# marian42/shapegan

Measured on AMD Instinct MI355X. Metric: GAN train steps/sec @32^3 voxels (train_wgan.py 5 critic + 1 generator updates, batch 64/GPU), higher is better.
Workload: dtype f32; 1 GPU; train_wgan.py 32^3 voxel WGAN, fp32, batch=64 synthetic SDF grids (BASELINE configs[1]); global_batch=64, per_gpu_batch=64, parallelism=dp1

## Files before the change

### shapegan_amd/csrc/conv3d.hip

```cpp
#include "mfma_tile.h"
#include <stdlib.h>

#include "conv_common.h"
#include "../../include/shapegan_hip.h"

namespace sg {

struct PatchCtx {
    int base;
    int mask;
    __device__ __forceinline__ void set(const ConvGeom& g, uint32_t pos) {
        int n, od, oh, ow;
        decode_pos(g, pos, n, od, oh, ow);
        const int id0 = 2 * od - 1, ih0 = 2 * oh - 1, iw0 = 2 * ow - 1;
        base = n * g.Cx * g.ID * g.IH * g.IW + (id0 * g.IH + ih0) * g.IW + iw0;
        int m = 0;
#pragma unroll
        for (int t = 0; t < 4; ++t) {
            if ((unsigned)(id0 + t) < (unsigned)g.ID) m |= 1 << t;
            if ((unsigned)(ih0 + t) < (unsigned)g.IH) m |= 1 << (4 + t);
            if ((unsigned)(iw0 + t) < (unsigned)g.IW) m |= 1 << (8 + t);
        }
        mask = m;
    }
// ... 655 lines not shown
                      false);
}
int sg_conv3d_k4s2p1_dgrad_keep(const float* dy, const float* w, const float* bias, float* dx, int batch, int Cin,
                                int Cin_total, int Cx, int Cout, int ID, int IH, int IW, int act, float slope,
                                void* workspace, size_t workspace_bytes, int weights_unchanged, hipStream_t stream) {
    return dgrad_call(dy, w, bias, dx, batch, Cin, Cin_total, Cx, Cout, ID, IH, IW, act, slope, workspace, workspace_bytes, stream,
                      weights_unchanged != 0);
}

int sg_conv3d_k4s2p1_pack_images(int n, const int* kinds, const float* const* weights, void* const* workspaces,
                                 const size_t* workspace_bytes, const int* dims, int* served, hipStream_t stream) {
    SG_CHECK_ARG(n > 0 && n <= 8 && kinds && weights && workspaces && workspace_bytes && dims && served);
    PackJobs jobs;
    static const float dummy = 0.f;
    for (int i = 0; i < n; ++i) {
        const int* d = dims + 8 * i;
        const int batch = d[0], Cin = d[1], Cin_total = d[2], Cx = d[3], Cout = d[4];
        served[i] = 0;
        SG_CHECK_ARG(weights[i] && batch > 0 && Cin > 0 && Cin <= Cin_total && Cin <= Cx && Cout > 0 && (kinds[i] == 0 || kinds[i] == 1));
        ConvGeom g;
        if (make_geom(g, d[5], d[6], d[7], Cx, Cout)) SG_FAIL(SG_ERR_ARG, "sg_conv3d_k4s2p1_pack_images: bad spatial dims");
        if (check_sizes(g, batch, "sg_conv3d_k4s2p1_pack_images")) return SG_ERR_ARG;
        if (Cin == 1) continue;
        int rc;
        if (kinds[i] == 0)
            rc = halo_fwd_try(&dummy, weights[i], nullptr, const_cast<float*>(&dummy), batch, Cin, Cin_total, g, Cout, SG_ACT_NONE, 0.f,
                              workspaces[i], workspace_bytes[i], stream, 0, 0, false, &jobs);
        else
            rc = halo_dgrad_try(&dummy, weights[i], nullptr, const_cast<float*>(&dummy), batch, Cin, Cin_total, g, Cout, SG_ACT_NONE, 0.f,
                                workspaces[i], workspace_bytes[i], stream, 0, false, &jobs);
        if (rc < 0) return rc;
        served[i] = rc == 1;
    }
    halo_pack_jobs_launch(jobs, stream);
    SG_CHECK_LAUNCH();
    return SG_OK;
}

long long sg_conv3d_k4s2p1_image_layout(int kind, const int* dims, size_t workspace_bytes) {
    if (!dims || (kind != 0 && kind != 1)) return 0;
    const int batch = dims[0], Cin = dims[1], Cin_total = dims[2], Cx = dims[3], Cout = dims[4];
    if (batch <= 0 || Cin <= 1 || Cin > Cin_total || Cin > Cx || Cout <= 0) return 0;
    ConvGeom g;
    if (make_geom(g, dims[5], dims[6], dims[7], Cx, Cout)) return 0;
    if ((long)batch * g.O3() >= (1L << 31) || (long)batch * g.I3() >= (1L << 31)) return 0;
    PackJobs jobs;
    static const float dummy = 0.f;
    char* const base = reinterpret_cast<char*>(uintptr_t(1) << 20);
    const int rc = kind == 0 ? halo_fwd_try(&dummy, &dummy, nullptr, const_cast<float*>(&dummy), batch, Cin, Cin_total, g, Cout, SG_ACT_NONE,
                                            0.f, base, workspace_bytes, nullptr, 0, 0, false, &jobs)
                             : halo_dgrad_try(&dummy, &dummy, nullptr, const_cast<float*>(&dummy), batch, Cin, Cin_total, g, Cout,
                                              SG_ACT_NONE, 0.f, base, workspace_bytes, nullptr, 0, false, &jobs);
    if (rc != 1 || jobs.n != 1) return 0;
    const PackJob& j = jobs.job[0];
    unsigned long long h = 1469598103934665603ull;
    const long long f[7] = {j.kind + 1, j.Cout, j.Cin_total, j.Cin, j.nt, (long long)(reinterpret_cast<char*>(j.wp) - base), 0x5347};
    for (long long v : f)
        for (int b = 0; b < 8; ++b) {
            h ^= (unsigned long long)(v >> (8 * b)) & 0xffull;
            h *= 1099511628211ull;
        }
    h &= 0x7fffffffffffffffull;
    return h ? (long long)h : 1;
}

int sg_conv3d_k4s2p1_dgrad_impl(const float* dy, const float* w, const float* bias, float* dx, int batch, int Cin,
                                int Cin_total, int Cx, int Cout, int ID, int IH, int IW, int act, float slope,
                                void* workspace, size_t workspace_bytes, int impl, hipStream_t stream) {
    SG_CHECK_ARG(dy && w && dx && batch > 0 && Cin > 0 && Cin <= Cin_total && Cin <= Cx && Cout > 0 && (impl & 1) &&
                 (impl == 1 || impl == 3 || impl == 9 || impl == 17 || impl == 33));
    ConvGeom g;
    if (make_geom(g, ID, IH, IW, Cx, Cout)) SG_FAIL(SG_ERR_ARG, "sg_conv3d_k4s2p1_dgrad_impl: bad spatial dims");
    if (check_sizes(g, batch, "sg_conv3d_k4s2p1_dgrad_impl")) return SG_ERR_ARG;
    const int rc = halo_dgrad_try(dy, w, bias, dx, batch, Cin, Cin_total, g, Cout, act, slope, workspace, workspace_bytes,
                                  stream, impl);
    if (rc != 1) SG_FAIL(SG_ERR_ARG, "sg_conv3d_k4s2p1_dgrad_impl: shape not eligible for the LDS-halo kernel");
    SG_CHECK_LAUNCH();
    return SG_OK;
}

int sg_conv3d_k4s2p1_wgrad_impl(const float* dy, const float* x, float* dw, int batch, int Cin, int Cin_total, int Cx,
                                int Cout, int ID, int IH, int IW, void* workspace, size_t workspace_bytes, int impl,
                                hipStream_t stream) {
    SG_CHECK_ARG(dy && x && dw && batch > 0 && Cin > 0 && Cin <= Cin_total && Cin <= Cx && Cout > 0 && impl == 1);
    ConvGeom g;
    if (make_geom(g, ID, IH, IW, Cx, Cout)) SG_FAIL(SG_ERR_ARG, "sg_conv3d_k4s2p1_wgrad_impl: bad spatial dims");
    if (check_sizes(g, batch, "sg_conv3d_k4s2p1_wgrad_impl")) return SG_ERR_ARG;
    const int rc = halo_wgrad_try(dy, x, dw, batch, Cin, Cin_total, g, Cout, workspace, workspace_bytes, stream, 1);
    if (rc != 1) SG_FAIL(SG_ERR_ARG, "sg_conv3d_k4s2p1_wgrad_impl: shape not eligible for the LDS-halo kernel");
    SG_CHECK_LAUNCH();
    return SG_OK;
}

int sg_conv3d_k4s2p1_wgrad_dy_image(int batch, int Cin, int Cout, int OD, int OH, int OW, size_t workspace_bytes, int* mt_total,
                                    long* nslice) {
    if (batch <= 0 || Cin <= 0 || Cout <= 0 || !mt_total || !nslice) return 0;
    ConvGeom g;
    if (make_geom(g, 2 * OD, 2 * OH, 2 * OW, Cin, Cout)) return 0;
    if (Cin == 1 && Cout <= 64) return 0;
    return halo_wgrad_dy_image_plan(batch, Cin, Cout, g, workspace_bytes, mt_total, nslice);
}
int sg_act_bwd_rowsum_pack8(const float* y, const float* dy, float* dz, float* rowsum, void* dz_image, long N, int C, long nslice,
                            int act, float slope, hipStream_t stream) {
    SG_CHECK_ARG(y && dy && dz && rowsum && dz_image && N > 0 && C > 0 && C % 128 == 0 && nslice == N * 8);
    SG_CHECK_ARG(act == SG_ACT_LEAKY || act == SG_ACT_RELU);
    SG_CHECK_ARG((((uintptr_t)y | (uintptr_t)dy | (uintptr_t)dz | (uintptr_t)dz_image) & 15) == 0);
    halo_act_bwd_pack8_launch(y, dy, dz, rowsum, dz_image, N * C, C, nslice, act, slope, stream);
    SG_CHECK_LAUNCH();
    return SG_OK;
}
int sg_conv3d_k4s2p1_wgrad_prepacked(const float* dy, const float* x, float* dw, int batch, int Cin, int Cin_total, int Cx,
                                     int Cout, int ID, int IH, int IW, void* workspace, size_t workspace_bytes, hipStream_t stream) {
    SG_CHECK_ARG(dy && x && dw && batch > 0 && Cin > 0 && Cin <= Cin_total && Cin <= Cx && Cout > 0);
    ConvGeom g;
    if (make_geom(g, ID, IH, IW, Cx, Cout)) SG_FAIL(SG_ERR_ARG, "sg_conv3d_k4s2p1_wgrad_prepacked: bad spatial dims");
    if (check_sizes(g, batch, "sg_conv3d_k4s2p1_wgrad_prepacked")) return SG_ERR_ARG;
    int mt;
    long ns;
    if (!halo_wgrad_dy_image_plan(batch, Cin, Cout, g, workspace_bytes, &mt, &ns))
        SG_FAIL(SG_ERR_ARG, "sg_conv3d_k4s2p1_wgrad_prepacked: this call is not served with a producer-written image");
    if (halo_wgrad_try(dy, x, dw, batch, Cin, Cin_total, g, Cout, workspace, workspace_bytes, stream, 0, true) != 1)
        SG_FAIL(SG_ERR_ARG, "sg_conv3d_k4s2p1_wgrad_prepacked: not served");
    SG_CHECK_LAUNCH();
    return SG_OK;
}

int sg_conv3d_k4s2p1_wgrad_act_eligible(int batch, int Cin, int Cout, int OD, int OH, int OW, int act) {
    const size_t x_bytes = ((size_t)batch * 8 * OD * OH * OW + (size_t)(2 * OH + 1) * 2 * OW + 4) * 4;
    const size_t dy_bytes = (size_t)batch * Cout * OD * OH * OW * 4;
    return Cin == 1 && Cout <= 64 && OW % 16 == 0 && (long)batch * OD * OH * OW >= 65536 && (act == SG_ACT_LEAKY || act == SG_ACT_RELU) &&
           x_bytes < (size_t)kBufRange && dy_bytes < (size_t)kBufRange && edge_enabled(4);
}
int sg_conv3d_k4s2p1_wgrad_act(const float* dy, const float* y, const float* x, float* dw, float* db, int batch, int Cin,
                               int Cin_total, int Cx, int Cout, int ID, int IH, int IW, int act, float slope, void* workspace,
                               size_t workspace_bytes, hipStream_t stream) {
    SG_CHECK_ARG(dy && y && x && dw && db && batch > 0 && Cin > 0 && Cin <= Cin_total && Cin <= Cx && Cout > 0);
    ConvGeom g;
    if (make_geom(g, ID, IH, IW, Cx, Cout)) SG_FAIL(SG_ERR_ARG, "sg_conv3d_k4s2p1_wgrad_act: spatial dims must be even and >= 2");
    if (check_sizes(g, batch, "sg_conv3d_k4s2p1_wgrad_act")) return SG_ERR_ARG;
    if (!sg_conv3d_k4s2p1_wgrad_act_eligible(batch, Cin, Cout, g.OD, g.OH, g.OW, act) ||
        edge_wgrad_try(dy, x, dw, batch, Cin, Cin_total, g, Cout, workspace, workspace ? workspace_bytes : 0, stream, 0, y, act, slope,
                       db) != 1)
        SG_FAIL(SG_ERR_ARG, "sg_conv3d_k4s2p1_wgrad_act: shape not served (see sg_conv3d_k4s2p1_wgrad_act_eligible) or workspace too small");
    SG_CHECK_LAUNCH();
    return SG_OK;
}

int sg_conv3d_k4s2p1_wgrad(const float* dy, const float* x, float* dw, int batch, int Cin, int Cin_total, int Cx,
                           int Cout, int ID, int IH, int IW, void* workspace, size_t workspace_bytes,
                           hipStream_t stream) {
    SG_CHECK_ARG(dy && x && dw && batch > 0 && Cin > 0 && Cin <= Cin_total && Cin <= Cx && Cout > 0);
    ConvGeom g;
    if (make_geom(g, ID, IH, IW, Cx, Cout)) SG_FAIL(SG_ERR_ARG, "sg_conv3d_k4s2p1_wgrad: spatial dims must be even and >= 2");
    if (check_sizes(g, batch, "sg_conv3d_k4s2p1_wgrad")) return SG_ERR_ARG;
    const long npos = (long)batch * g.O3();
    if (Cin == 1 && edge_enabled(4) &&
        edge_wgrad_try(dy, x, dw, batch, Cin, Cin_total, g, Cout, workspace, workspace ? workspace_bytes : 0, stream) == 1) {
        SG_CHECK_LAUNCH();
        return SG_OK;
    }
    {
        const int rc = halo_wgrad_try(dy, x, dw, batch, Cin, Cin_total, g, Cout, workspace, workspace ? workspace_bytes : 0,
                                      stream, 0);
        if (rc < 0) return rc;
        if (rc == 1) {
            SG_CHECK_LAUNCH();
            return SG_OK;
        }
    }
    WgradDyLoader la;
    la.dy = dy;
// ... 69 lines not shown
```

### shapegan_amd/csrc/conv3d_halo.hip

```cpp
#include "conv_common.h"

#ifndef SG_RING
#define SG_RING 8
#endif
#ifndef SG_ABLATE
#define SG_ABLATE 0
#endif

namespace sg {

constexpr int kHD = 4, kHH = 18, kHWF = 18;
constexpr int kHWH = 10;
constexpr int kROWH = 2 * kHWH;
constexpr int kROWD = kHH * kROWH;
constexpr int kHS = kHD * kROWD;
constexpr int kCC = 4;

struct HaloFwdArgs {
    const float* x;
    const float4* wp;
    const float* bias;
    float* y;
    ConvGeom g;
    int Cin, Cout;
// ... 1038 lines not shown
                for (int t = 0; t < 2; ++t) a_cur[t] = aring[gq][t];
                int gi = (st + 1) * 8 + gq;
                gi = gi < G ? gi : G - 1;
#pragma unroll
                for (int t = 0; t < 2; ++t) aring[gq][t] = buf_load4(ares[t], avoff, (unsigned)gi * 1024u);
                float b[2][4];
#pragma unroll
                for (int tn = 0; tn < 2; ++tn)
#pragma unroll
                    for (int j = 0; j < 4; ++j) b[tn][j] = bq[tn][j];
                if (gq + 1 < 8) {
#pragma unroll
                    for (int tn = 0; tn < 2; ++tn) {
                        const lds_float* hb = bb[CUR][tn][(gq + 1) >> 2] + 2 * ((gq + 1) & 3) * kROWH;
                        bq[tn][0] = hb[0];
                        bq[tn][1] = hb[2];
                        bq[tn][2] = hb[4];
                        bq[tn][3] = hb[6];
                    }
                }
#pragma unroll
                for (int f = 0; f < NF; ++f) {
                    if (f * 4 / NF == gq) fv[f] = copy_load(f);
                    if (f * 4 / NF + 4 == gq) sdst[f % (kWNF / 2)][NXT * (NCH * kWHS) + (f / (kWNF / 2)) * kWHS] = fv[f];
                }
                __builtin_amdgcn_sched_barrier(0);
#pragma unroll
                for (int j = 0; j < 4; ++j) {
                    const float a0 = j == 0 ? a_cur[0].x : (j == 1 ? a_cur[0].y : (j == 2 ? a_cur[0].z : a_cur[0].w));
                    const float a1 = j == 0 ? a_cur[1].x : (j == 1 ? a_cur[1].y : (j == 2 ? a_cur[1].z : a_cur[1].w));
                    acc[0][0] = __builtin_amdgcn_mfma_f32_32x32x2f32(a0, b[0][j], acc[0][0], 0, 0, 0);
                    acc[1][0] = __builtin_amdgcn_mfma_f32_32x32x2f32(a1, b[0][j], acc[1][0], 0, 0, 0);
                    acc[0][1] = __builtin_amdgcn_mfma_f32_32x32x2f32(a0, b[1][j], acc[0][1], 0, 0, 0);
                    acc[1][1] = __builtin_amdgcn_mfma_f32_32x32x2f32(a1, b[1][j], acc[1][1], 0, 0, 0);
                }
                __builtin_amdgcn_sched_barrier(0);
            }
            __syncthreads();
        };
        for (int st = 0; st + 1 < nst; st += 2) {
            stage(IntTag<0>(), st);
            stage(IntTag<1>(), st + 1);
        }
        if (nst & 1) stage(IntTag<0>(), nst - 1);
    }

    float* out = a.ws + (long)split * a.Cout * a.ldw;
#pragma unroll
    for (int tn = 0; tn < 2; ++tn) {
        const int col = wn * 64 + tn * 32 + r;
        const int ci = ci0 + (col >> 6);
        if (ci >= a.Cin) continue;
        const long cbase = (long)ci * 64 + (col & 63);
#pragma unroll
        for (int t = 0; t < 2; ++t) {
#pragma unroll
            for (int q = 0; q < 16; ++q) {
                const int co = (mt0 + wm * 2 + t) * 32 + (q & 3) + 8 * (q >> 2) + 4 * kpar;
                if (co < a.Cout) out[(long)co * a.ldw + cbase] = acc[t][tn][q];
            }
        }
    }
}

__global__ void __launch_bounds__(256) pack_wgrad_dy4_kernel(const float* __restrict__ dy, float4* __restrict__ ap, int Cout,
                                                             int MT, int nslice) {
    const long total = (long)MT * nslice * 8 * 64;
    for (long e = (long)blockIdx.x * 256 + threadIdx.x; e < total; e += (long)gridDim.x * 256) {
        const int lane = (int)(e & 63);
        const int gq = (int)((e >> 6) & 7);
        const long q = e >> 9;
        const long sl = q % nslice;
        const int mt = (int)(q / nslice);
        const int co = mt * 32 + (lane & 31);
        float4 v = make_float4(0.f, 0.f, 0.f, 0.f);
        if (co < Cout) {
            const float* src = dy + (sl * Cout + co) * 64 + (gq >> 1) * 16 + (gq & 1) * 8 + (lane >> 5);
            v = make_float4(src[0], src[2], src[4], src[6]);
        }
        ap[e] = v;
    }
}

__global__ void __launch_bounds__(256) conv_wgrad_halo4_kernel(HaloWgradArgs a) {
    constexpr int kBUF = 2 * k4CH;
    extern __shared__ __attribute__((aligned(16))) float wbox[];
    lds_float* const wl = (lds_float*)wbox;
    const int tid = threadIdx.x, lane = tid & 63;
    const int wave = __builtin_amdgcn_readfirstlane(tid >> 6);
    const int wm = wave >> 1, wn = wave & 1, r = lane & 31, kpar = lane >> 5;
    const int ci0 = blockIdx.x * 2, mt0 = blockIdx.y * 4, split = blockIdx.z;
    const int s_beg = split * a.per_split, s_end = min(a.nslice, s_beg + a.per_split);
    const int nst = s_end - s_beg;

    f32x16 acc[2][2];
#pragma unroll
    for (int i = 0; i < 2; ++i)
#pragma unroll
        for (int j = 0; j < 2; ++j)
#pragma unroll
            for (int q = 0; q < 16; ++q) acc[i][j][q] = 0.f;

    for (int e = tid; e < 2 * kBUF; e += 256) wl[e] = 0.f;

    if (nst > 0) {
        const lds_float* bb[2][2][4];
#pragma unroll
        for (int tn = 0; tn < 2; ++tn) {
            const int tap = tn * 32 + r, kd = tap >> 4, kh = (tap >> 2) & 3, kw = tap & 3;
            const int lb = wn * k4CH + kd * k4PLANE + kh * k4ROW + (kw & 1) * k4HALF + (kw >> 1) + kpar;
#pragma unroll
            for (int b = 0; b < 2; ++b)
#pragma unroll
                for (int od = 0; od < 4; ++od) {
                    bb[b][tn][od] = wl + b * kBUF + lb + od * (2 * k4PLANE);
                    pin_vgpr(bb[b][tn][od]);
                }
        }
        unsigned voff[4];
        lds_float* sdst[4];
#pragma unroll
        for (int f = 0; f < 4; ++f) {
            const int e = tid + 256 * f, c = e >> 9, idx = e & 511;
            const int id = idx >> 6, ih = (idx >> 3) & 7, iw = idx & 7;
            voff[f] = (ci0 + c) < a.Cin ? (unsigned)e * 4u : kBufOutside;
            sdst[f] = wl + c * k4CH + (id + 1) * k4PLANE + (ih + 1) * k4ROW + ((iw + 1) & 1) * k4HALF + ((iw + 1) >> 1);
            pin_vgpr(voff[f]);
            pin_vgpr(sdst[f]);
        }
        __amdgpu_buffer_rsrc_t ares[2];
#pragma unroll
        for (int t = 0; t < 2; ++t) ares[t] = make_rsrc(a.ap + ((long)(mt0 + wm * 2 + t) * a.nslice + s_beg) * 8 * 64);
        const unsigned avoff = lane * 16;
        const long slice_floats = (long)a.g.Cx * 512;
        const float* xb = a.x + (long)s_beg * slice_floats + (long)ci0 * 512;
        const int G = nst * 8;
        constexpr int kRing = 8;
        float fv[4];
        __syncthreads();
        {
            const __amdgpu_buffer_rsrc_t xres = make_rsrc(xb);
#pragma unroll
            for (int f = 0; f < 4; ++f) fv[f] = buf_load(xres, voff[f], 0);
        }
        float4 aring[kRing][2];
#pragma unroll
        for (int u = 0; u < kRing; ++u)
#pragma unroll
            for (int t = 0; t < 2; ++t) aring[u][t] = buf_load4(ares[t], avoff, (unsigned)(u < G ? u : G - 1) * 1024u);
#pragma unroll
        for (int f = 0; f < 4; ++f) *sdst[f] = fv[f];
        __syncthreads();

        auto stage = [&](auto tag, int st) {
            constexpr int CUR = decltype(tag)::value, NXT = CUR ^ 1;
            const int snext = st + 1 < nst ? st + 1 : st;
            const __amdgpu_buffer_rsrc_t xres = make_rsrc(xb + (long)snext * slice_floats);
            float bq[2][4];
#pragma unroll
            for (int tn = 0; tn < 2; ++tn) {
                const lds_float* hb = bb[CUR][tn][0];
                bq[tn][0] = hb[0];
                bq[tn][1] = hb[2];
                bq[tn][2] = hb[2 * k4ROW];
                bq[tn][3] = hb[2 * k4ROW + 2];
            }
            __builtin_amdgcn_sched_barrier(0);
#pragma unroll
            for (int gq = 0; gq < 8; ++gq) {
                float4 a_cur[2];
#pragma unroll
                for (int t = 0; t < 2; ++t) a_cur[t] = aring[gq][t];
                int gi = (st + 1) * 8 + gq;
                gi = gi < G ? gi : G - 1;
#pragma unroll
                for (int t = 0; t < 2; ++t) aring[gq][t] = buf_load4(ares[t], avoff, (unsigned)gi * 1024u);
                float b[2][4];
#pragma unroll
                for (int tn = 0; tn < 2; ++tn)
#pragma unroll
                    for (int j = 0; j < 4; ++j) b[tn][j] = bq[tn][j];
                if (gq + 1 < 8) {
#pragma unroll
                    for (int tn = 0; tn < 2; ++tn) {
                        const lds_float* hb = bb[CUR][tn][(gq + 1) >> 1] + ((gq + 1) & 1) * (4 * k4ROW);
                        bq[tn][0] = hb[0];
                        bq[tn][1] = hb[2];
                        bq[tn][2] = hb[2 * k4ROW];
                        bq[tn][3] = hb[2 * k4ROW + 2];
                    }
                }
                if (gq < 4) fv[gq] = buf_load(xres, voff[gq], 0);
                else sdst[gq - 4][NXT * kBUF] = fv[gq - 4];
                __builtin_amdgcn_sched_barrier(0);
#pragma unroll
                for (int j = 0; j < 4; ++j) {
                    const float a0 = j == 0 ? a_cur[0].x : (j == 1 ? a_cur[0].y : (j == 2 ? a_cur[0].z : a_cur[0].w));
                    const float a1 = j == 0 ? a_cur[1].x : (j == 1 ? a_cur[1].y : (j == 2 ? a_cur[1].z : a_cur[1].w));
                    acc[0][0] = __builtin_amdgcn_mfma_f32_32x32x2f32(a0, b[0][j], acc[0][0], 0, 0, 0);
                    acc[1][0] = __builtin_amdgcn_mfma_f32_32x32x2f32(a1, b[0][j], acc[1][0], 0, 0, 0);
                    acc[0][1] = __builtin_amdgcn_mfma_f32_32x32x2f32(a0, b[1][j], acc[0][1], 0, 0, 0);
                    acc[1][1] = __builtin_amdgcn_mfma_f32_32x32x2f32(a1, b[1][j], acc[1][1], 0, 0, 0);
                }
                __builtin_amdgcn_sched_barrier(0);
            }
            __syncthreads();
        };
        for (int st = 0; st + 1 < nst; st += 2) {
            stage(IntTag<0>(), st);
            stage(IntTag<1>(), st + 1);
        }
        if (nst & 1) stage(IntTag<0>(), nst - 1);
    }

    float* out = a.ws + (long)split * a.Cout * a.ldw;
#pragma unroll
    for (int tn = 0; tn < 2; ++tn) {
        const int col = wn * 64 + tn * 32 + r;
        const int ci = ci0 + (col >> 6);
        if (ci >= a.Cin) continue;
        const long cbase = (long)ci * 64 + (col & 63);
#pragma unroll
        for (int t = 0; t < 2; ++t) {
#pragma unroll
            for (int q = 0; q < 16; ++q) {
                const int co = (mt0 + wm * 2 + t) * 32 + (q & 3) + 8 * (q >> 2) + 4 * kpar;
                if (co < a.Cout) out[(long)co * a.ldw + cbase] = acc[t][tn][q];
            }
        }
    }
}

__global__ void __launch_bounds__(256) wgrad_halo_finalize_kernel(const float* __restrict__ ws, float* __restrict__ dw,
                                                                  int Cout, int ncol, long ldw, int nsplit) {
    const long total = (long)Cout * ncol, total4 = total >> 2;
    for (long e4 = (long)blockIdx.x * 256 + threadIdx.x; e4 < total4; e4 += (long)gridDim.x * 256) {
        const f32x4* p = reinterpret_cast<const f32x4*>(ws) + e4;
        f32x4 v = {0.f, 0.f, 0.f, 0.f};
        int s = 0;
        for (; s + 3 < nsplit; s += 4) {
            const f32x4 a0 = p[(long)s * total4], a1 = p[(long)(s + 1) * total4], a2 = p[(long)(s + 2) * total4],
                        a3 = p[(long)(s + 3) * total4];
            v += a0;
            v += a1;
            v += a2;
            v += a3;
        }
        for (; s < nsplit; ++s) v += p[(long)s * total4];
        const long e = e4 << 2;
        const long co = e / ncol, c = e - co * ncol;
        *reinterpret_cast<f32x4*>(dw + co * ldw + c) = v;
    }
}

static bool wgrad_mode4(const ConvGeom& g) { return g.OD == 4 && g.OH == 4 && g.OW == 4; }

static bool wgrad_rows64(const ConvGeom& g, int Cin, int Cout) {
    return !wgrad_mode4(g) && Cout <= 64 && Cin >= 4 && Cin % 4 == 0;
}
static void wgrad_halo_plan(int batch, const ConvGeom& g, int Cin, int Cout, int& nslice, int& nsplit, int& mtiles) {
    nslice = wgrad_mode4(g) ? batch : batch * g.OD * (g.OH / 8) * (g.OW / 8);
    const bool rows64 = wgrad_rows64(g, Cin, Cout);
    mtiles = rows64 ? (Cout + 63) / 64 : (Cout + 127) / 128;
    const int ntiles = (rows64 ? Cin / 4 : (Cin + 1) / 2) * mtiles;
    nsplit = (512 + ntiles - 1) / ntiles;
    if (nsplit > nslice / 4) nsplit = nslice / 4 > 0 ? nslice / 4 : 1;
    if (nsplit < 1) nsplit = 1;
}

size_t halo_wgrad_workspace_bytes(int batch, int Cin, int Cout, int OD, int OH, int OW) {
    if ((OH % 8 != 0 || OW % 8 != 0) && !(OD == 4 && OH == 4 && OW == 4)) return 0;
    ConvGeom g;
    g.OD = OD;
    g.OH = OH;
    g.OW = OW;
    int nslice, nsplit, mtiles;
    g.ID = 2 * OD;
    g.IH = 2 * OH;
    g.IW = 2 * OW;
    wgrad_halo_plan(batch, g, Cin, Cout, nslice, nsplit, mtiles);
    const size_t pack = (size_t)mtiles * 4 * nslice * 8 * 64 * sizeof(float4);
    const size_t part = (size_t)nsplit * Cout * Cin * 64 * sizeof(float);
    return pack + part + 256;
}

int halo_wgrad_dy_image_plan(int batch, int Cin, int Cout, const ConvGeom& g, size_t workspace_bytes, int* mt_total, long* nslice_out) {
    const bool mode4 = wgrad_mode4(g);
    if (!(mode4 || (g.OD == 8 && g.OH == 8 && g.OW == 8)) || Cout % 128 != 0 || Cin < 2) return 0;
    if ((long)batch * g.Cx * g.ID * g.IH * g.IW >= (1L << 31) || (long)2 * g.ID * g.IH * g.IW * 4 >= (1L << 26)) return 0;
    int nslice, nsplit, mtiles;
    wgrad_halo_plan(batch, g, Cin, Cout, nslice, nsplit, mtiles);
    const int ntiles = ((Cin + 1) / 2) * mtiles;
    if (Cout <= 64 || (long)ntiles * nsplit < 384) return 0;
    if (workspace_bytes < halo_wgrad_workspace_bytes(batch, Cin, Cout, g.OD, g.OH, g.OW)) return 0;
    *mt_total = mtiles * 4;
    *nslice_out = nslice;
    return 1;
}

__global__ void __launch_bounds__(256) act_bwd_pack8_kernel(const float* __restrict__ y, const float* __restrict__ dy,
                                                            float* __restrict__ dz, float* __restrict__ rowsum,
                                                            float4* __restrict__ ap, long rows, int C, long nslice, int act, float slope) {
    const long row = (long)blockIdx.x * 4 + (threadIdx.x >> 6);
    if (row >= rows) return;
    const int lane = threadIdx.x & 63;
    const long base = row * 512 + lane * 8;
    const f32x4 y0 = *reinterpret_cast<const f32x4*>(y + base), y1 = *reinterpret_cast<const f32x4*>(y + base + 4);
    const f32x4 g0 = *reinterpret_cast<const f32x4*>(dy + base), g1 = *reinterpret_cast<const f32x4*>(dy + base + 4);
    f32x4 z0, z1;
#pragma unroll
    for (int j = 0; j < 4; ++j) {
        z0[j] = act == SG_ACT_LEAKY ? (y0[j] > 0.f ? g0[j] : g0[j] * slope) : (y0[j] > 0.f ? g0[j] : 0.f);
        z1[j] = act == SG_ACT_LEAKY ? (y1[j] > 0.f ? g1[j] : g1[j] * slope) : (y1[j] > 0.f ? g1[j] : 0.f);
    }
    *reinterpret_cast<f32x4*>(dz + base) = z0;
    *reinterpret_cast<f32x4*>(dz + base + 4) = z1;
    const float s = sg_wave_sum(((z0[0] + z0[1]) + (z0[2] + z0[3])) + ((z1[0] + z1[1]) + (z1[2] + z1[3])));
    if (lane == 0) rowsum[row] = s;
    const long n = row / C;
    const int co = (int)(row - n * C), mt = co >> 5, r = co & 31, od = lane >> 3, oh = lane & 7;
    const long e = (((long)mt * nslice + n * 8 + od) * 8 + oh) * 64 + r;
    ap[e] = make_float4(z0[0], z0[2], z1[0], z1[2]);
    ap[e + 32] = make_float4(z0[1], z0[3], z1[1], z1[3]);
}
int halo_act_bwd_pack8_launch(const float* y, const float* dy, float* dz, float* rowsum, void* ap, long rows, int C, long nslice,
                              int act, float slope, hipStream_t stream) {
    hipLaunchKernelGGL(act_bwd_pack8_kernel, dim3((unsigned)((rows + 3) / 4)), dim3(256), 0, stream, y, dy, dz, rowsum, (float4*)ap,
                       rows, C, nslice, act, slope);
    return 1;
}

int halo_wgrad_try(const float* dy, const float* x, float* dw, int batch, int Cin, int Cin_total, const ConvGeom& g, int Cout,
                   void* workspace, size_t workspace_bytes, hipStream_t stream, int force, bool dy_packed) {
    const bool mode4 = wgrad_mode4(g);
    if ((!mode4 && (g.OW % 8 != 0 || g.OH % 8 != 0)) || Cin < 2 || Cout < 32) return 0;
    if ((long)batch * g.Cx * g.ID * g.IH * g.IW >= (1L << 31)) return 0;
    if ((long)2 * g.ID * g.IH * g.IW * 4 >= (1L << 26)) return 0;
    int nslice, nsplit, mtiles;
    wgrad_halo_plan(batch, g, Cin, Cout, nslice, nsplit, mtiles);
    const bool rows64 = wgrad_rows64(g, Cin, Cout) && (long)4 * g.ID * g.IH * g.IW * 4 < (1L << 26);
    if (wgrad_rows64(g, Cin, Cout) && !rows64) return 0;
    const int ntiles = (rows64 ? Cin / 4 : (Cin + 1) / 2) * mtiles;
    if (!force && ((Cout <= 64 && !rows64) || (long)ntiles * nsplit < 384)) return 0;
    const size_t need = halo_wgrad_workspace_bytes(batch, Cin, Cout, g.OD, g.OH, g.OW);
    if (!workspace || workspace_bytes < need) return 0;
    const int per_split = (nslice + nsplit - 1) / nsplit;
    nsplit = (nslice + per_split - 1) / per_split;

    const FastDiv dntw(mode4 ? 1 : g.OW / 8), dnth(mode4 ? 1 : g.OH / 8), dOD(g.OD);
    float4* ap = (float4*)workspace;
    const size_t pack_floats4 = (size_t)mtiles * 4 * nslice * 8 * 64;
    float* part = (float*)(ap + pack_floats4);
    if (!dy_packed) {
        int blocks = (int)((pack_floats4 + 255) / 256);
        if (blocks > 8192) blocks = 8192;
        if (mode4)
            hipLaunchKernelGGL(pack_wgrad_dy4_kernel, dim3(blocks), dim3(256), 0, stream, dy, ap, Cout, mtiles * 4, nslice);
        else
            hipLaunchKernelGGL(pack_wgrad_dy_kernel, dim3(blocks), dim3(256), 0, stream, dy, ap, g, Cout, rows64 ? mtiles * 2 : mtiles * 4,
                               nslice, dntw, dnth, dOD);
    }
    HaloWgradArgs a;
    a.ap = ap;
    a.x = x;
    a.g = g;
    a.Cin = Cin;
    a.Cout = Cout;
    a.nslice = nslice;
    a.per_split = per_split;
    a.mt_total = rows64 ? mtiles * 2 : mtiles * 4;
    a.dntw = dntw;
    a.dnth = dnth;
    a.dOD = dOD;
    const bool direct = nsplit == 1;
    a.ws = direct ? dw : part;
    a.ldw = direct ? (long)Cin_total * 64 : (long)Cin * 64;
    if (mode4) {
        hipLaunchKernelGGL(conv_wgrad_halo4_kernel, dim3((Cin + 1) / 2, mtiles, nsplit), dim3(256),
                           (size_t)2 * 2 * k4CH * sizeof(float), stream, a);
    } else {
        if (rows64) {
            const size_t lds = (size_t)2 * 4 * kWHS * sizeof(float);
            hipLaunchKernelGGL(conv_wgrad_halo_kernel<4>, dim3(Cin / 4, mtiles, nsplit), dim3(256), lds, stream, a);
        } else {
            const size_t lds = (size_t)2 * 2 * kWHS * sizeof(float);
            hipLaunchKernelGGL(conv_wgrad_halo_kernel<2>, dim3((Cin + 1) / 2, mtiles, nsplit), dim3(256), lds, stream, a);
        }
    }
    if (!direct) {
        const long total = (long)Cout * Cin * 64;
        int fb = (int)((total / 4 + 255) / 256);
        if (fb > 2048) fb = 2048;
        hipLaunchKernelGGL(wgrad_halo_finalize_kernel, dim3(fb), dim3(256), 0, stream, (const float*)part, dw, Cout, Cin * 64,
                           (long)Cin_total * 64, nsplit);
    }
    return 1;
}

}
```

### shapegan_amd/ops.py

```python
import ctypes
import weakref

import torch
from torch.autograd import Function
from torch.autograd.function import once_differentiable

from . import lib as L
from .lib import ACT_LEAKY, ACT_NONE, ACT_RELU, ACT_SIGMOID, ACT_TANH, check, f32c, ptr, stream, workspace


def _lib():
    return L.load()


def conv_fwd_raw(x, w, bias, act=ACT_NONE, slope=0.0, keep=False):
    N, Cx, D, H, W = x.shape
    Co, Ct = w.shape[0], w.shape[1]
    if Cx > Ct:
        raise RuntimeError("conv: input has %d channels, weight expects %d" % (Cx, Ct))
    ptr(x)
    L.reset_call_state()
    y = torch.empty((N, Co, D // 2, H // 2, W // 2), dtype=torch.float32, device=x.device)
    lib = _lib()
    nb = lib.sg_conv3d_k4s2p1_fwd_workspace_bytes(N, Cx, Co, D // 2, H // 2, W // 2)
# ... 150 lines not shown
def _param_grad_out(param, shape, device):
    dst = L.grad_destination(param, shape) if param is not None else None
    return dst if dst is not None else torch.empty(shape, dtype=torch.float32, device=device)


def conv_wgrad_raw(dy, x, ct, out=None):
    N, Co, OD, OH, OW = dy.shape
    Cx = x.shape[1]
    if x.shape[0] != N or x.shape[2] != 2 * OD:
        raise RuntimeError("conv wgrad: shape mismatch")
    if out is not None:
        dw = out
        if Cx < ct:
            dw.zero_()
    elif Cx < ct:
        dw = torch.zeros((Co, ct, 4, 4, 4), dtype=torch.float32, device=dy.device)
    else:
        dw = torch.empty((Co, ct, 4, 4, 4), dtype=torch.float32, device=dy.device)
    lib = _lib()
    nb = min(lib.sg_conv3d_k4s2p1_wgrad_workspace_bytes(N, Cx, Co, OD, OH, OW), _WGRAD_WS_CAP)
    ws = workspace("splitk", nb, dy.device)
    check(lib.sg_conv3d_k4s2p1_wgrad(ptr(dy), ptr(x), ptr(dw), N, Cx, ct, Cx, Co, 2 * OD, 2 * OH, 2 * OW, ptr(ws),
                                     ws.numel(), stream()), "conv3d_wgrad")
    return dw


def _wgrad_dy_image(N, Cx, Co, O, device):
    if device.type != "cuda":
        return None
    lib = _lib()
    nb = min(lib.sg_conv3d_k4s2p1_wgrad_workspace_bytes(N, Cx, Co, O, O, O), _WGRAD_WS_CAP)
    ws = workspace("splitk", nb, device)
    mt, ns = ctypes.c_int(0), ctypes.c_long(0)
    if not lib.sg_conv3d_k4s2p1_wgrad_dy_image(N, Cx, Co, O, O, O, ws.numel(), ctypes.byref(mt), ctypes.byref(ns)):
        return None
    return ws, mt.value, ns.value


def conv_wgrad_prepacked_raw(dy, x, ct, ws, out=None):
    N, Co = dy.shape[0], dy.shape[1]
    Cx = x.shape[1]
    dw = out if out is not None else torch.empty((Co, ct, 4, 4, 4), dtype=torch.float32, device=dy.device)
    if Cx < ct:
        raise RuntimeError("conv_wgrad_prepacked: partial input channels are not served")
    check(_lib().sg_conv3d_k4s2p1_wgrad_prepacked(ptr(dy), ptr(x), ptr(dw), N, Cx, ct, Cx, Co, x.shape[2], x.shape[3], x.shape[4],
                                                  ptr(ws), ws.numel(), stream()), "conv3d_wgrad_prepacked")
    return dw


def act_bwd_rowsum_pack8_raw(y, dy, act, slope, ws, nslice, gb_out=None):
    y, dy = f32c(y), f32c(dy)
    N, C = y.shape[0], y.shape[1]
    lib = _lib()
    dz = torch.empty_like(y)
    rows = torch.empty(N * C, dtype=torch.float32, device=y.device)
    check(lib.sg_act_bwd_rowsum_pack8(ptr(y), ptr(dy), ptr(dz), ptr(rows), ptr(ws), N, C, nslice, act, slope, stream()),
          "act_bwd_rowsum_pack8")
    gb = torch.empty(C, dtype=torch.float32, device=y.device) if gb_out is None else gb_out
    check(lib.sg_colsum(ptr(rows), ptr(gb), N, C, C, stream()), "colsum")
    return dz, gb


def conv_wgrad_act_raw(dy, y, x, act, slope, dw_out=None, db_out=None):
    N, Co, OD, OH, OW = dy.shape
    Cx = x.shape[1]
    dw = dw_out if dw_out is not None else torch.empty((Co, Cx, 4, 4, 4), dtype=torch.float32, device=dy.device)
    db = db_out if db_out is not None else torch.empty(Co, dtype=torch.float32, device=dy.device)
    lib = _lib()
    nb = min(lib.sg_conv3d_k4s2p1_wgrad_workspace_bytes(N, Cx, Co, OD, OH, OW), _WGRAD_WS_CAP)
    ws = workspace("splitk", nb, dy.device)
    check(lib.sg_conv3d_k4s2p1_wgrad_act(ptr(dy), ptr(y), ptr(x), ptr(dw), ptr(db), N, Cx, Cx, Cx, Co, 2 * OD, 2 * OH, 2 * OW, act,
                                         slope, ptr(ws), ws.numel(), stream()), "conv3d_wgrad_act")
    return dw, db


def _wgrad_act_served(x, w, y, act):
    lib = _lib()
    N, Cx, Co = x.shape[0], x.shape[1], w.shape[0]
    if not lib.sg_conv3d_k4s2p1_wgrad_act_eligible(N, Cx, Co, y.shape[2], y.shape[3], y.shape[4], act):
        return False
    return lib.sg_conv3d_k4s2p1_wgrad_workspace_bytes(N, Cx, Co, y.shape[2], y.shape[3], y.shape[4]) <= _WGRAD_WS_CAP


def conv_wgrad_halo_raw(dy, x, ct):
    N, Co, OD, OH, OW = dy.shape
    Cx = x.shape[1]
    dw = torch.zeros((Co, ct, 4, 4, 4), dtype=torch.float32, device=dy.device)
    lib = _lib()
    ws = workspace("splitk", lib.sg_conv3d_k4s2p1_wgrad_workspace_bytes(N, Cx, Co, OD, OH, OW), dy.device)
    check(lib.sg_conv3d_k4s2p1_wgrad_impl(ptr(dy), ptr(x), ptr(dw), N, Cx, ct, Cx, Co, 2 * OD, 2 * OH, 2 * OW, ptr(ws),
                                          ws.numel(), 1, stream()), "conv3d_wgrad_impl")
    return dw


def gemm_raw(a, ta, b, tb, bias_j=None, bias_shift=0, act=ACT_NONE, slope=0.0, out=None, a_off=0, b_off=0, M=None,
             N=None, K=None, lda=None, ldb=None, ldc=None, c_off=0):
    lda = a.shape[-1] if lda is None else lda
    ldb = b.shape[-1] if ldb is None else ldb
    if M is None:
        M = a.shape[1] if ta else a.shape[0]
    if K is None:
        K = a.shape[0] if ta else a.shape[1]
    if N is None:
        N = b.shape[0] if tb else b.shape[1]
    sai, sak = (1, lda) if ta else (lda, 1)
    sbk, sbj = (1, ldb) if tb else (ldb, 1)
    if out is None:
        out = torch.empty((M, N), dtype=torch.float32, device=a.device)
    ldc = out.shape[-1] if ldc is None else ldc
    lib = _lib()
    nb = min(lib.sg_gemm_workspace_bytes(M, N), _WGRAD_WS_CAP)
    ws = workspace("splitk", nb, a.device)
    check(lib.sg_gemm(ptr(a) + 4 * a_off, sai, sak, ptr(b) + 4 * b_off, sbk, sbj, ptr(out) + 4 * c_off, ldc, 1, None,
                      ptr(bias_j), bias_shift, M, N, K, act, slope, ptr(ws), ws.numel(), stream()), "gemm")
    return out


def gemm_nt_raw(a, b, out, M, N, K, lda, ldb, ldc, a_off=0, b_off=0, c_off=0):
    lib = _lib()
    ws = workspace("gemm_nt", lib.sg_gemm_nt_workspace_bytes(M, N, K), a.device)
    check(lib.sg_gemm_nt(ptr(a) + 4 * a_off, lda, ptr(b) + 4 * b_off, ldb, ptr(out) + 4 * c_off, ldc, M, N, K, ptr(ws),
                         ws.numel(), stream()), "gemm_nt")
    return out


def act_bwd_raw(y, dy, act, slope):
    dx = torch.empty_like(y)
    check(_lib().sg_act_bwd(ptr(y), ptr(dy), ptr(dx), y.numel(), act, slope, stream()), "act_bwd")
    return dx


def act_bwd_rowsum_raw(y, dy, act, slope, gb_out=None):
    y, dy = f32c(y), f32c(dy)
    N, C = y.shape[0], y.shape[1]
    S = y.numel() // (N * C)
    lib = _lib()
    dz = torch.empty_like(y)
    rows = torch.empty(N * C, dtype=torch.float32, device=y.device)
    check(lib.sg_act_bwd_rowsum(ptr(y), ptr(dy), ptr(dz), ptr(rows), N * C, S, act, slope, stream()), "act_bwd_rowsum")
    gb = torch.empty(C, dtype=torch.float32, device=y.device) if gb_out is None else gb_out
    check(lib.sg_colsum(ptr(rows), ptr(gb), N, C, C, stream()), "colsum")
    return dz, gb


def act_fwd_raw(x, act, slope):
    y = torch.empty_like(x)
    check(_lib().sg_act_fwd(ptr(x), ptr(y), x.numel(), act, slope, stream()), "act_fwd")
    return y


def channel_sum_raw(g, out=None):
    N, C = g.shape[0], g.shape[1]
    S = g.numel() // (N * C)
    lib = _lib()
    if out is None:
        out = torch.empty(C, dtype=torch.float32, device=g.device)
    if S == 1:
        check(lib.sg_colsum(ptr(g), ptr(out), N, C, C, stream()), "colsum")
        return out
    tmp = torch.empty(N * C, dtype=torch.float32, device=g.device)
    check(lib.sg_rowsum(ptr(g), ptr(tmp), N * C, S, S, stream()), "rowsum")
    check(lib.sg_colsum(ptr(tmp), ptr(out), N, C, C, stream()), "colsum")
    return out


class ActBwd(Function):

    @staticmethod
    def forward(ctx, y, dy, act, slope):
        y, dy = f32c(y), f32c(dy)
        ctx.act, ctx.slope = act, slope
        ctx.save_for_backward(y)
        ctx.dy = dy if act in (ACT_TANH, ACT_SIGMOID) else None
        return act_bwd_raw(y, dy, act, slope)
# ... 1718 lines not shown
```

Before: 60.53 steps/s.

## Skip padding-only MFMA tiles in 4^3 wgrad halo kernel by remapping waves

Restructures the 4^3 wgrad halo kernel so each wave owns one 32-row Cout tile and all four kd tap planes, instead of a 2x2 split of Cout tiles and tap halves. With that layout, MFMAs and LDS reads for kd/od combinations that only touch zero padding (kd=0 with the first depth slab, kd=3 with the last) can be skipped at compile time. A DENSE template variant keeps the old full computation and is selectable through impl 3. The change cuts wasted MFMA work on the border planes. In exchange, each wave loads fewer A tiles but more B operands, which changes register pressure and the output write pattern.

Result: no change. 61.14 steps/s, median of 6 (+1.0%).

```diff
diff --git a/shapegan_amd/csrc/conv3d.hip b/shapegan_amd/csrc/conv3d.hip
--- a/shapegan_amd/csrc/conv3d.hip
+++ b/shapegan_amd/csrc/conv3d.hip
@@ -761,11 +761,12 @@
 int sg_conv3d_k4s2p1_wgrad_impl(const float* dy, const float* x, float* dw, int batch, int Cin, int Cin_total, int Cx,
                                 int Cout, int ID, int IH, int IW, void* workspace, size_t workspace_bytes, int impl,
                                 hipStream_t stream) {
-    SG_CHECK_ARG(dy && x && dw && batch > 0 && Cin > 0 && Cin <= Cin_total && Cin <= Cx && Cout > 0 && impl == 1);
+    SG_CHECK_ARG(dy && x && dw && batch > 0 && Cin > 0 && Cin <= Cin_total && Cin <= Cx && Cout > 0 && (impl == 1 || impl == 3));
     ConvGeom g;
     if (make_geom(g, ID, IH, IW, Cx, Cout)) SG_FAIL(SG_ERR_ARG, "sg_conv3d_k4s2p1_wgrad_impl: bad spatial dims");
+    if (impl == 3 && !(g.OD == 4 && g.OH == 4 && g.OW == 4)) SG_FAIL(SG_ERR_ARG, "sg_conv3d_k4s2p1_wgrad_impl: impl 3 exists on 4^3 grids only");
     if (check_sizes(g, batch, "sg_conv3d_k4s2p1_wgrad_impl")) return SG_ERR_ARG;
-    const int rc = halo_wgrad_try(dy, x, dw, batch, Cin, Cin_total, g, Cout, workspace, workspace_bytes, stream, 1);
+    const int rc = halo_wgrad_try(dy, x, dw, batch, Cin, Cin_total, g, Cout, workspace, workspace_bytes, stream, impl);
     if (rc != 1) SG_FAIL(SG_ERR_ARG, "sg_conv3d_k4s2p1_wgrad_impl: shape not eligible for the LDS-halo kernel");
     SG_CHECK_LAUNCH();
     return SG_OK;
diff --git a/shapegan_amd/csrc/conv3d_halo.hip b/shapegan_amd/csrc/conv3d_halo.hip
--- a/shapegan_amd/csrc/conv3d_halo.hip
+++ b/shapegan_amd/csrc/conv3d_halo.hip
@@ -1144,40 +1144,41 @@
     }
 }
 
+template <bool DENSE>
 __global__ void __launch_bounds__(256) conv_wgrad_halo4_kernel(HaloWgradArgs a) {
     constexpr int kBUF = 2 * k4CH;
     extern __shared__ __attribute__((aligned(16))) float wbox[];
     lds_float* const wl = (lds_float*)wbox;
     const int tid = threadIdx.x, lane = tid & 63;
     const int wave = __builtin_amdgcn_readfirstlane(tid >> 6);
-    const int wm = wave >> 1, wn = wave & 1, r = lane & 31, kpar = lane >> 5;
+    const int r = lane & 31, kpar = lane >> 5;
     const int ci0 = blockIdx.x * 2, mt0 = blockIdx.y * 4, split = blockIdx.z;
     const int s_beg = split * a.per_split, s_end = min(a.nslice, s_beg + a.per_split);
     const int nst = s_end - s_beg;
-
-    f32x16 acc[2][2];
-#pragma unroll
-    for (int i = 0; i < 2; ++i)
-#pragma unroll
-        for (int j = 0; j < 2; ++j)
-#pragma unroll
-            for (int q = 0; q < 16; ++q) acc[i][j][q] = 0.f;
+    auto live = [](int kd, int gq) constexpr { return DENSE || !((kd == 0 && gq < 2) || (kd == 3 && gq >= 6)); };
+
+    f32x16 acc[4];
+#pragma unroll
+    for (int i = 0; i < 4; ++i)
+#pragma unroll
+        for (int q = 0; q < 16; ++q) acc[i][q] = 0.f;
 
     for (int e = tid; e < 2 * kBUF; e += 256) wl[e] = 0.f;
 
     if (nst > 0) {
-        const lds_float* bb[2][2][4];
-#pragma unroll
-        for (int tn = 0; tn < 2; ++tn) {
-            const int tap = tn * 32 + r, kd = tap >> 4, kh = (tap >> 2) & 3, kw = tap & 3;
-            const int lb = wn * k4CH + kd * k4PLANE + kh * k4ROW + (kw & 1) * k4HALF + (kw >> 1) + kpar;
+        const lds_float* bb[2][4][4];
+        {
+            const int c = r >> 4, kh = (r >> 2) & 3, kw = r & 3;
+            const int lb = c * k4CH + kh * k4ROW + (kw & 1) * k4HALF + (kw >> 1) + kpar;
 #pragma unroll
             for (int b = 0; b < 2; ++b)
 #pragma unroll
-                for (int od = 0; od < 4; ++od) {
-                    bb[b][tn][od] = wl + b * kBUF + lb + od * (2 * k4PLANE);
-                    pin_vgpr(bb[b][tn][od]);
-                }
+                for (int kd = 0; kd < 4; ++kd)
+#pragma unroll
+                    for (int od = 0; od < 4; ++od) {
+                        bb[b][kd][od] = wl + b * kBUF + lb + kd * k4PLANE + od * (2 * k4PLANE);
+                        if (live(kd, 2 * od)) pin_vgpr(bb[b][kd][od]);
+                    }
         }
         unsigned voff[4];
         lds_float* sdst[4];
@@ -1190,9 +1191,7 @@
             pin_vgpr(voff[f]);
             pin_vgpr(sdst[f]);
         }
-        __amdgpu_buffer_rsrc_t ares[2];
-#pragma unroll
-        for (int t = 0; t < 2; ++t) ares[t] = make_rsrc(a.ap + ((long)(mt0 + wm * 2 + t) * a.nslice + s_beg) * 8 * 64);
+        const __amdgpu_buffer_rsrc_t ares = make_rsrc(a.ap + ((long)(mt0 + wave) * a.nslice + s_beg) * 8 * 64);
         const unsigned avoff = lane * 16;
         const long slice_floats = (long)a.g.Cx * 512;
         const float* xb = a.x + (long)s_beg * slice_floats + (long)ci0 * 512;
@@ -1205,11 +1204,9 @@
 #pragma unroll
             for (int f = 0; f < 4; ++f) fv[f] = buf_load(xres, voff[f], 0);
         }
-        float4 aring[kRing][2];
-#pragma unroll
-        for (int u = 0; u < kRing; ++u)
-#pragma unroll
-            for (int t = 0; t < 2; ++t) aring[u][t] = buf_load4(ares[t], avoff, (unsigned)(u < G ? u : G - 1) * 1024u);
+        float4 aring[kRing];
+#pragma unroll
+        for (int u = 0; u < kRing; ++u) aring[u] = buf_load4(ares, avoff, (unsigned)(u < G ? u : G - 1) * 1024u);
 #pragma unroll
         for (int f = 0; f < 4; ++f) *sdst[f] = fv[f];
         __syncthreads();
@@ -1218,38 +1215,37 @@
             constexpr int CUR = decltype(tag)::value, NXT = CUR ^ 1;
             const int snext = st + 1 < nst ? st + 1 : st;
             const __amdgpu_buffer_rsrc_t xres = make_rsrc(xb + (long)snext * slice_floats);
-            float bq[2][4];
-#pragma unroll
-            for (int tn = 0; tn < 2; ++tn) {
-                const lds_float* hb = bb[CUR][tn][0];
-                bq[tn][0] = hb[0];
-                bq[tn][1] = hb[2];
-                bq[tn][2] = hb[2 * k4ROW];
-                bq[tn][3] = hb[2 * k4ROW + 2];
+            float bq[4][4] = {};
+#pragma unroll
+            for (int kd = 0; kd < 4; ++kd) {
+                if (!live(kd, 0)) continue;
+                const lds_float* hb = bb[CUR][kd][0];
+                bq[kd][0] = hb[0];
+                bq[kd][1] = hb[2];
+                bq[kd][2] = hb[2 * k4ROW];
+                bq[kd][3] = hb[2 * k4ROW + 2];
             }
             __builtin_amdgcn_sched_barrier(0);
 #pragma unroll
             for (int gq = 0; gq < 8; ++gq) {
-                float4 a_cur[2];
-#pragma unroll
-                for (int t = 0; t < 2; ++t) a_cur[t] = aring[gq][t];
+                const float4 a_cur = aring[gq];
                 int gi = (st + 1) * 8 + gq;
                 gi = gi < G ? gi : G - 1;
-#pragma unroll
-                for (int t = 0; t < 2; ++t) aring[gq][t] = buf_load4(ares[t], avoff, (unsigned)gi * 1024u);
-                float b[2][4];
-#pragma unroll
-                for (int tn = 0; tn < 2; ++tn)
-#pragma unroll
-                    for (int j = 0; j < 4; ++j) b[tn][j] = bq[tn][j];
+                aring[gq] = buf_load4(ares, avoff, (unsigned)gi * 1024u);
+                float b[4][4];
+#pragma unroll
+                for (int kd = 0; kd < 4; ++kd)
+#pragma unroll
+                    for (int j = 0; j < 4; ++j) b[kd][j] = bq[kd][j];
                 if (gq + 1 < 8) {
 #pragma unroll
-                    for (int tn = 0; tn < 2; ++tn) {
-                        const lds_float* hb = bb[CUR][tn][(gq + 1) >> 1] + ((gq + 1) & 1) * (4 * k4ROW);
-                        bq[tn][0] = hb[0];
-                        bq[tn][1] = hb[2];
-                        bq[tn][2] = hb[2 * k4ROW];
-                        bq[tn][3] = hb[2 * k4ROW + 2];
+                    for (int kd = 0; kd < 4; ++kd) {
+                        if (!live(kd, gq + 1)) continue;
+                        const lds_float* hb = bb[CUR][kd][(gq + 1) >> 1] + ((gq + 1) & 1) * (4 * k4ROW);
+                        bq[kd][0] = hb[0];
+                        bq[kd][1] = hb[2];
+                        bq[kd][2] = hb[2 * k4ROW];
+                        bq[kd][3] = hb[2 * k4ROW + 2];
                     }
                 }
                 if (gq < 4) fv[gq] = buf_load(xres, voff[gq], 0);
@@ -1257,12 +1253,10 @@
                 __builtin_amdgcn_sched_barrier(0);
 #pragma unroll
                 for (int j = 0; j < 4; ++j) {
-                    const float a0 = j == 0 ? a_cur[0].x : (j == 1 ? a_cur[0].y : (j == 2 ? a_cur[0].z : a_cur[0].w));
-                    const float a1 = j == 0 ? a_cur[1].x : (j == 1 ? a_cur[1].y : (j == 2 ? a_cur[1].z : a_cur[1].w));
-                    acc[0][0] = __builtin_amdgcn_mfma_f32_32x32x2f32(a0, b[0][j], acc[0][0], 0, 0, 0);
-                    acc[1][0] = __builtin_amdgcn_mfma_f32_32x32x2f32(a1, b[0][j], acc[1][0], 0, 0, 0);
-                    acc[0][1] = __builtin_amdgcn_mfma_f32_32x32x2f32(a0, b[1][j], acc[0][1], 0, 0, 0);
-                    acc[1][1] = __builtin_amdgcn_mfma_f32_32x32x2f32(a1, b[1][j], acc[1][1], 0, 0, 0);
+                    const float av = j == 0 ? a_cur.x : (j == 1 ? a_cur.y : (j == 2 ? a_cur.z : a_cur.w));
+#pragma unroll
+                    for (int kd = 0; kd < 4; ++kd)
+                        if (live(kd, gq)) acc[kd] = __builtin_amdgcn_mfma_f32_32x32x2f32(av, b[kd][j], acc[kd], 0, 0, 0);
                 }
                 __builtin_amdgcn_sched_barrier(0);
             }
@@ -1276,18 +1270,15 @@
     }
 
     float* out = a.ws + (long)split * a.Cout * a.ldw;
-#pragma unroll
-    for (int tn = 0; tn < 2; ++tn) {
-        const int col = wn * 64 + tn * 32 + r;
-        const int ci = ci0 + (col >> 6);
-        if (ci >= a.Cin) continue;
-        const long cbase = (long)ci * 64 + (col & 63);
-#pragma unroll
-        for (int t = 0; t < 2; ++t) {
+    const int ci = ci0 + (r >> 4);
+    if (ci < a.Cin) {
+#pragma unroll
+        for (int kd = 0; kd < 4; ++kd) {
+            const long cbase = (long)ci * 64 + kd * 16 + (r & 15);
 #pragma unroll
             for (int q = 0; q < 16; ++q) {
-                const int co = (mt0 + wm * 2 + t) * 32 + (q & 3) + 8 * (q >> 2) + 4 * kpar;
-                if (co < a.Cout) out[(long)co * a.ldw + cbase] = acc[t][tn][q];
+                const int co = (mt0 + wave) * 32 + (q & 3) + 8 * (q >> 2) + 4 * kpar;
+                if (co < a.Cout) out[(long)co * a.ldw + cbase] = acc[kd][q];
             }
         }
     }
@@ -1438,8 +1429,12 @@
     a.ws = direct ? dw : part;
     a.ldw = direct ? (long)Cin_total * 64 : (long)Cin * 64;
     if (mode4) {
-        hipLaunchKernelGGL(conv_wgrad_halo4_kernel, dim3((Cin + 1) / 2, mtiles, nsplit), dim3(256),
-                           (size_t)2 * 2 * k4CH * sizeof(float), stream, a);
+        if (force & 2)
+            hipLaunchKernelGGL(conv_wgrad_halo4_kernel<true>, dim3((Cin + 1) / 2, mtiles, nsplit), dim3(256),
+                               (size_t)2 * 2 * k4CH * sizeof(float), stream, a);
+        else
+            hipLaunchKernelGGL(conv_wgrad_halo4_kernel<false>, dim3((Cin + 1) / 2, mtiles, nsplit), dim3(256),
+                               (size_t)2 * 2 * k4CH * sizeof(float), stream, a);
     } else {
         if (rows64) {
             const size_t lds = (size_t)2 * 4 * kWHS * sizeof(float);
diff --git a/shapegan_amd/ops.py b/shapegan_amd/ops.py
--- a/shapegan_amd/ops.py
+++ b/shapegan_amd/ops.py
@@ -256,14 +256,14 @@
     return lib.sg_conv3d_k4s2p1_wgrad_workspace_bytes(N, Cx, Co, y.shape[2], y.shape[3], y.shape[4]) <= _WGRAD_WS_CAP
 
 
-def conv_wgrad_halo_raw(dy, x, ct):
+def conv_wgrad_halo_raw(dy, x, ct, impl=1):
     N, Co, OD, OH, OW = dy.shape
     Cx = x.shape[1]
     dw = torch.zeros((Co, ct, 4, 4, 4), dtype=torch.float32, device=dy.device)
     lib = _lib()
     ws = workspace("splitk", lib.sg_conv3d_k4s2p1_wgrad_workspace_bytes(N, Cx, Co, OD, OH, OW), dy.device)
     check(lib.sg_conv3d_k4s2p1_wgrad_impl(ptr(dy), ptr(x), ptr(dw), N, Cx, ct, Cx, Co, 2 * OD, 2 * OH, 2 * OW, ptr(ws),
-                                          ws.numel(), 1, stream()), "conv3d_wgrad_impl")
+                                          ws.numel(), impl, stream()), "conv3d_wgrad_impl")
     return dw
 
 
```
